# rickenator/steganosaurus

Hardware: AMD Instinct MI355X
Metric: MPixels/s embed+extract round-trip (RGB 2D-FFT fwd+inv) (higher is better)
Workload: dtype f32

## Files before the change

steganosaurus_amd/csrc/tfft_kernels.hip:

```cpp
#include <hip/hip_runtime.h>
#include <float.h>
#include <math.h>
#include <stdint.h>

#include <type_traits>

#include "tfft_fft.h"
#include "tfft_device.h"
#include "tfft_kernels.h"

#ifndef TFFT_WAVES_PER_EU
#define TFFT_WAVES_PER_EU(n) __attribute__((amdgpu_waves_per_eu(n)))
#endif
#ifndef TFFT_COLS_WAVES
#define TFFT_COLS_WAVES(logl) ((logl) >= 8 ? 4 : 1)
#endif
#ifndef TFFT_COLS_PF_MAXLOG
#define TFFT_COLS_PF_MAXLOG 7
#endif
#ifndef TFFT_COLS_PFEMIT
#define TFFT_COLS_PFEMIT 0
#endif
#ifndef TFFT_ROWS_LAZY_LOG
#define TFFT_ROWS_LAZY_LOG 11
// ... 636 lines not shown
            dstw[3 * g + 1] = G1 | (B1 << 8) | (R2 << 16) | (G2 << 24);
            dstw[3 * g + 2] = B2 | (R3 << 8) | (G3 << 16) | (B3 << 24);
        }
    } else {
        auto get = [&](int off) -> unsigned {
            const int n = off / 3, ch = off - 3 * n;
            float v = ldsf[2 * lay.idx(n >> 1, ch - plane0) + (n & 1)];
            if (P.center && ((n + y) & 1)) v = -v;
            return quantise_u8(v + (cov ? (float)cov[off] : P.bias));
        };
        if (PPB == 3) {
            const int head = (int)((4 - ((uintptr_t)dst & 3)) & 3);
            for (int o = tid; o < head && o < nbytes; o += nthr) dst[o] = (uint8_t)get(o);
            const int nwords = nbytes > head ? (nbytes - head) / 4 : 0;
            uint32_t* dstw = reinterpret_cast<uint32_t*>(dst + head);
            for (int w = tid; w < nwords; w += nthr) {
                const int o = head + 4 * w;
                dstw[w] = get(o) | (get(o + 1) << 8) | (get(o + 2) << 16) | (get(o + 3) << 24);
            }
            for (int o = head + 4 * nwords + tid; o < nbytes; o += nthr) dst[o] = (uint8_t)get(o);
        } else if ((P.W & 1) == 0) {
            const float s0 = (P.center && (y & 1)) ? -1.0f : 1.0f, s1 = P.center ? -s0 : s0;
            uint8_t* d1 = dst + plane0;
            constexpr int NP = imax(1, (M + T * PPB - 1) / (T * PPB));
            uint32_t cv[2 * NP];
            if (cov) {
#pragma unroll
                for (int i = 0; i < NP; i++) {
                    const uint8_t* a = cov + plane0 + 6 * imin(tid + i * nthr, (P.W >> 1) - 1);
                    cv[2 * i] = cover_word(a);
                    cv[2 * i + 1] = cover_word(a + 3);
                }
            }
#pragma unroll
            for (int i = 0; i < NP; i++) {
                const int m = tid + i * nthr;
                if (m >= (P.W >> 1)) break;
                const float2 v = lds[lay.idx(m, 0)];
                d1[6 * m] = (uint8_t)quantise_u8(s0 * v.x + (cov ? (float)cover_pick(cv[2 * i], cov + plane0 + 6 * m) : P.bias));
                d1[6 * m + 3] = (uint8_t)quantise_u8(s1 * v.y + (cov ? (float)cover_pick(cv[2 * i + 1], cov + plane0 + 6 * m + 3) : P.bias));
            }
        } else {
            for (int n = tid; n < P.W; n += nthr) dst[3 * n + plane0] = (uint8_t)get(3 * n + plane0);
        }
    }
}

__device__ __forceinline__ unsigned opaque_u32(unsigned v) {
#if defined(__HIPCC__)
    asm volatile("" : "+v"(v));
#endif
    return v;
}
constexpr int cols_threads(int logl) { return imax(256, 16 * ((1 << logl) / elems_for(1 << logl))); }
__device__ __forceinline__ int read_bit_value(float2 v, const EmbedParams& P, int p, const float* __restrict__ jitter, uint64_t j);

__device__ __forceinline__ unsigned frame_bit(const uint8_t* __restrict__ header, const uint8_t* __restrict__ payload, uint64_t i);
template <int LOGL, int SIGN, int MODE = COLS_PLAIN, bool DC = false, bool TW = false, bool FULL = false, bool PH = false, bool PI = false>
__global__ void __launch_bounds__(cols_threads(LOGL)) TFFT_WAVES_PER_EU((MODE == COLS_EMIT && TFFT_COLS_PFEMIT) ? 1 : (FULL ? TFFT_COLS_WAVES(LOGL) : imin(2, TFFT_COLS_WAVES(LOGL)))) k_fft_cols(const float2* in, float2* out, const float2* __restrict__ tw,
                           ColParams P) {
    constexpr int L = 1 << LOGL, E = elems_for(L), T = L / E, C = 16;
    constexpr bool STAT = stat_mode(MODE), FUSED = (MODE == COLS_STAT_EMBED);
    const int c = threadIdx.x, t = threadIdx.y, gl = (FUSED && T * C >= 256) ? 0 : (int)threadIdx.z;
    const int g = (MODE == COLS_PLAIN && SIGN > 0 && FULL && P.g_step > 1) ? (int)(blockIdx.y * blockDim.z + gl) * P.g_step + P.g_off
                                                                            : (int)(blockIdx.y * blockDim.z + gl);
    const int img = blockIdx.z / 3, plane = blockIdx.z - 3 * img;
    const size_t plane_off = (size_t)img * P.img_stride + (size_t)plane * P.plane_stride;
    float2* lds = reinterpret_cast<float2*>(tfft_smem) + (size_t)gl * L * C;
    LayColumns lay{C};

    if (MODE == COLS_PLAIN && SIGN > 0 && P.gate) {
        const SelectState* gs = P.gate + 3 * img;
        if (gs[0].fast && gs[1].fast && gs[2].fast && gs[0].n_amb <= TFFT_AMB_CAP && gs[1].n_amb <= TFFT_AMB_CAP && gs[2].n_amb <= TFFT_AMB_CAP) return;
    }
    const int ts = (MODE == COLS_PLAIN && SIGN > 0 && P.tile_step > 1) ? P.tile_step : 1;
    const int toff = ts > 1 ? P.tile_off : 0;
    const int tile0 = blockIdx.x * P.tiles_per_block;
    const int ntiles = ((P.M + C - 1) / C - toff + ts - 1) / ts;
    const int tile1 = (tile0 + P.tiles_per_block < ntiles) ? tile0 + P.tiles_per_block : ntiles;
    const int rows_in_max = P.in_a * (L - 1) + P.in_b * (P.G - 1);
    const bool in_full = (rows_in_max < P.in_rows) && (P.M % C == 0) && (P.G % (int)blockDim.z == 0);
    const unsigned voff_in = (unsigned)((P.in_a * t + P.in_b * g) * P.M + c) * 8u;
    const size_t stride_in = (size_t)P.in_a * T * P.M * sizeof(float2);
    const char* in_bytes = reinterpret_cast<const char*>(in + plane_off);
    const int oM = ts > 1 ? P.out_M : P.M;
    const unsigned voff_out = (unsigned)((P.out_a * t + P.out_b * g) * oM + c) * 8u;
    const size_t stride_out = (size_t)P.out_a * T * oM * sizeof(float2);
    char* out_bytes = reinterpret_cast<char*>(out + (ts > 1 ? (size_t)img * P.out_img_stride + (size_t)plane * P.out_plane_stride : plane_off));
    char* m2_bytes = reinterpret_cast<char*>(reinterpret_cast<float*>(out + (size_t)img * P.img_stride) + (size_t)plane * P.plane_stride);
    auto load_tile = [&](int tile, float2 (&v)[E]) {
        if (in_full) {
            const char* tb = in_bytes + (size_t)(imin(tile, ntiles - 1) * ts + toff) * (C * sizeof(float2));
            const unsigned vo = opaque_u32(voff_in);
#pragma unroll
            for (int m = 0; m < E; m++) v[m] = *reinterpret_cast<const float2*>(tb + m * stride_in + vo);
        } else {
            const int col = imin((tile * ts + toff) * C + c, P.M - 1);
            const float2* src = in + plane_off;
            const int gc = imin(g, P.G - 1), to = (int)opaque_u32((unsigned)t);
#pragma unroll
            for (int m = 0; m < E; m++) {
                const int row = imin(P.in_a * (to + m * T) + P.in_b * gc, P.in_rows - 1);
                v[m] = src[(unsigned)(row * P.M + col)];
            }
        }
    };
    auto tile_mask = [&](int tile, float2 (&v)[E]) {
        if (in_full) return;
        const bool active = ((tile * ts + toff) * C + c < P.M) && (g < P.G);
#pragma unroll
        for (int m = 0; m < E; m++) {
            const int row = P.in_a * (t + m * T) + P.in_b * g;
            if (!(active && row < P.in_rows)) v[m] = make_float2(0.f, 0.f);
        }
    };
    constexpr bool PF = (LOGL <= TFFT_COLS_PF_MAXLOG || (MODE == COLS_EMIT && TFFT_COLS_PFEMIT)) && !embed_mode(MODE);
    float2 u[E], un[E];
    float2 awc = make_float2(0.f, 0.f), awn = make_float2(0.f, 0.f);
    auto load_aw = [&](int tile) -> float2 { const int col = (tile * ts + toff) * C + c; return (DC && col < P.M) ? P.dc_aw[col] : make_float2(0.f, 0.f); };
    if (PF) { load_tile(tile0, u); awc = load_aw(tile0); }
    const int out_rows = (MODE == COLS_ROWLIMIT) ? imin(P.out_rows, *P.last_row_dev + 1) : P.out_rows;
    float2* lds_ah = reinterpret_cast<float2*>(tfft_smem) + (size_t)blockDim.z * L * C + (size_t)gl * L;
    float2* lds_wo = FUSED ? lds_ah : reinterpret_cast<float2*>(tfft_smem) + (size_t)blockDim.z * L * (C + (DC ? 1 : 0)) + (size_t)gl * L;
    auto fu_load_wo = [&]() -> float2 { return twload<-1>(tw, (int)((opaque_u32((unsigned)(t * C + c)) * (unsigned)g) & (unsigned)(P.PH - 1))); };
    auto fu_load_ah = [&]() -> float2 { return P.dc_ah[(unsigned)P.out_a * opaque_u32((unsigned)(t * C + c)) + (unsigned)(P.out_b * g)]; };
    if (FUSED && !DC) lds_wo[t * C + c] = fu_load_wo();
    if (DC) {
        for (int k = t * C + c; k < L; k += T * C) {
            const int row = (SIGN > 0) ? P.out_a * k + P.out_b * g : P.in_a * k + P.in_b * g;
            lds_ah[k] = (g < P.G && row < P.PH) ? P.dc_ah[row] : make_float2(0.f, 0.f);
        }
    }
    if (TW) {
        for (int k = t * C + c; k < L; k += T * C) lds_wo[k] = twload<SIGN>(tw, (k * g) & (P.PH - 1));
    }
    constexpr int NOFF = 16;
    constexpr bool TWL = (LOGL >= TFFT_COLS_LDS_TW_LOG) || FUSED;
    float2 W[TWL ? 1 : tw_regs<L, E>()];
    float2* lds_tw = reinterpret_cast<float2*>(tfft_smem) + (size_t)blockDim.z * L * (C + (DC || FUSED ? 1 : 0) + (TW ? 1 : 0));
    float2* lds_aw = lds_tw + (TWL ? L : 0) + gl * C;
    if (TWL) {
        const int tws = P.PH >> LOGL;
        for (int k = (gl * T + t) * C + c; k < L; k += blockDim.z * T * C) lds_tw[k] = tw[k * tws];
    } else {
        fft_prefetch_twiddles<L, E, SIGN>(W, t, tw, P.PH >> LOGL);
    }
#ifndef TFFT_EMBED_NE9
#ifndef TFFT_STAT_LDS_LOG
#define TFFT_STAT_LDS_LOG 9
#endif
#ifndef TFFT_STAT_SLOTS
#define TFFT_STAT_SLOTS 193
#endif
#define TFFT_EMBED_NE9 4
#endif
    constexpr int NE = (LOGL >= 9) ? (embed_mode(MODE) ? (LOGL == 9 ? TFFT_EMBED_NE9 : 2) : 4) : 2;
    struct EmEntry { TileBin tb; float2 f; unsigned bit, live; };
    EmEntry enC[NE], enN[NE];
    const int em_tid = t * C + c, em_nthr = T * C;
    unsigned* lds_eo = reinterpret_cast<unsigned*>(lds_tw + (TWL ? L : 0) + blockDim.z * C) + gl * (NOFF + 2);
    if (MODE == COLS_READ || embed_mode(MODE) || MODE == COLS_EMIT || STAT) {
        const unsigned b0 = (unsigned)(((PI ? (int)blockIdx.z : plane) * P.G + (g < P.G ? g : 0)) * ntiles);
        for (int i = em_tid; i <= NOFF; i += em_nthr) lds_eo[i] = P.rd_off[b0 + (unsigned)imin(tile0 + i, ntiles)];
    }
    unsigned* lds_hist = reinterpret_cast<unsigned*>(tfft_smem + P.hist_lds_off);
    const bool hist_on = (MODE == COLS_PLAIN && SIGN > 0 && FULL) && P.hist_sel != nullptr;
    if (hist_on)
        for (int i = (gl * T + t) * C + c; i < 4096; i += (int)(blockDim.x * blockDim.y * blockDim.z)) lds_hist[i] = 0;
    lds_barrier();
    auto em_range = [&](int tile, unsigned& e0, unsigned& e1) {
        const int i = imin(tile - tile0, NOFF - 1);
        e0 = lds_eo[i]; e1 = lds_eo[i + 1];
        if (!(tile < tile1 && g < P.G)) e1 = e0;
    };
    auto has_bins = [&](int tile) -> bool {
        if (MODE != COLS_READ || blockDim.z > 1) return true;
        unsigned e0, e1;
        em_range(tile, e0, e1);
        return e1 > e0;
    };
    const float2* em_fl = P.em_fl + (size_t)img * P.em_n;
    const uint8_t* em_pb = P.em_pb + (size_t)img * P.em_n;
    auto em_entries = [&](int tile, EmEntry (&en)[NE], bool with_value, bool with_bit) {
        unsigned e0, e1;
        em_range(tile, e0, e1);
#pragma unroll
        for (int i = 0; i < NE; i++) {
            const unsigned e = e0 + (unsigned)(em_tid + i * em_nthr);
            en[i].live = e < e1 ? 1u : 0u;
            const unsigned ec = en[i].live ? e : 0u;
            en[i].tb = P.rd_bins[ec];
            if (with_value) en[i].f = em_fl[ec];
            if (with_bit) en[i].bit = em_pb[ec];
        }
    };
    const float em_medp = (MODE == COLS_EMBED && PH && P.em_med) ? fmaxf(1e-12f, P.em_med[3 * img + plane]) : 1.f;
    auto em_delta = [&](float2 f, unsigned bit, unsigned conj, unsigned e) -> float2 {
        if (MODE == COLS_EMBED_D) return f;
        const float mag = fmaxf(1e-12f, mag_of(f));
        float ca = P.em_cos, sa = P.em_sin;
        if (MODE == COLS_EMBED && PH && P.em_med) sincosf(P.em_alpha * fminf(2.f, fmaxf(0.5f, mag / em_medp)), &sa, &ca);
        float2 nv = make_float2(mag * ca, bit ? mag * sa : -mag * sa);
        if (PH && P.em_jp) nv = cmul(nv, P.em_jp[e]);
        if (conj) nv = cconj(nv);
        return csub(nv, f);
    };
    const int st_lin = (gl * T + t) * C + c, st_wave = st_lin >> 6;
    unsigned* st_wbuf = lds_eo + (blockDim.z - gl) * (NOFF + 2) + st_wave * TFFT_STAT_SLOTS;
    SelectState* st_s = STAT ? P.st_sel + 3 * img + plane : nullptr;
    const unsigned st_lo = STAT ? st_s->lo : 0u, st_span = STAT ? st_s->hi - st_lo : 0u, st_base = st_lo << 19;
    const float st_t2lo = STAT ? fmaxf(st_s->t2_lo, 0.f) : 0.f, st_t2hi = STAT ? fmaxf(st_s->t2_hi, 0.f) : 0.f;
    unsigned* st_out = STAT ? P.st_cand + ((size_t)img * 3 + plane) * P.st_cand_stride : nullptr;
    float* st_ambo = STAT ? P.st_amb + ((size_t)img * 3 + plane) * TFFT_AMB_CAP : nullptr;
    unsigned st_below = 0, st_capcount = 0, st_nstaged = 0;
    const unsigned st_span_raw = st_span >= 8192u ? 0xFFFFFFFFu : ((st_span << 19) | 0x7FFFFu);
    const unsigned st_span_b = st_base > 0x7F800000u ? 0u : (st_span_raw < 0x7F800000u - st_base ? st_span_raw : 0x7F800000u - st_base);
    const unsigned st_aspan = (STAT && P.st_shi >= P.st_slo) ? P.st_shi - P.st_slo : 0u;
    const unsigned st_t2lo_b = __float_as_uint(st_t2lo), st_t2win = __float_as_uint(st_t2hi) - st_t2lo_b;
    unsigned* st_region = st_out + (size_t)(((blockIdx.y * gridDim.x + blockIdx.x) * ((blockDim.x * blockDim.y * blockDim.z + 63) >> 6)) + st_wave) * P.st_resv;
    if (STAT && blockIdx.x == 0 && blockIdx.y == 0 && st_lin == 0) st_s->cand_fixed = P.st_cand_fixed;
    unsigned st_used = 0;
    auto st_fill = [&]() {
        for (unsigned i = st_used + (st_lin & 63); i < P.st_resv; i += 64) st_region[i] = TFFT_CAND_HOLE;
    };
    auto st_flush = [&]() {
        const unsigned lane = st_lin & 63;
        WaveSync::sync();
        const unsigned room = P.st_resv - st_used, n1 = st_nstaged < room ? st_nstaged : room;
        for (unsigned i = lane; i < n1; i += 64) st_region[st_used + i] = st_wbuf[i];
        st_used += n1;
        if (st_nstaged > n1) {
            const unsigned rest = st_nstaged - n1;
            unsigned base = 0;
            if (lane == 0) base = atomicAdd(&st_s->n_cand, rest);
            base = __builtin_amdgcn_readfirstlane(base);
            if ((size_t)P.st_cand_fixed + base + rest <= P.st_cand_stride)
                for (unsigned i = lane; i < rest; i += 64) st_out[(size_t)P.st_cand_fixed + base + i] = st_wbuf[n1 + i];
        }
        WaveSync::sync();
        st_nstaged = 0;
    };
    if (embed_mode(MODE)) em_entries(tile0, enC, true, true);
    if (PF && (MODE == COLS_EMIT || STAT || MODE == COLS_READ)) em_entries(tile0, enC, false, FUSED);
    for (int tile = tile0; tile < tile1; tile++) {
        if (!PF && !embed_mode(MODE)) {
            if (!has_bins(tile)) continue;
            load_tile(tile, u); awc = load_aw(tile);
            if (MODE == COLS_EMIT || MODE == COLS_READ) em_entries(tile, enC, false, false);
        }
        if (PF) { const int nt = (tile + 1 < tile1 && has_bins(tile + 1)) ? tile + 1 : tile; load_tile(nt, un); awn = load_aw(nt); }
        if (PF && (MODE == COLS_EMIT || STAT || MODE == COLS_READ)) em_entries(tile + 1, enN, false, FUSED);
        if (embed_mode(MODE)) {
            bool hb = true;
            if (blockDim.z == 1) { unsigned e0, e1; em_range(tile, e0, e1); hb = e1 > e0; }
            em_entries(tile + 1, enN, true, true);
            if (hb) {
#pragma unroll
                for (int m = 0; m < E; m++) lds[lay.idx(t + m * T, c)] = make_float2(0.f, 0.f);
                lds_barrier();
                unsigned pe0 = 0;
                if (PH) { unsigned pe1; em_range(tile, pe0, pe1); }
#pragma unroll
                for (int i = 0; i < NE; i++)
                    if (enC[i].live && enC[i].bit < 2u)
                        lds[lay.idx(enC[i].tb.k, enC[i].tb.c)] = em_delta(enC[i].f, enC[i].bit, enC[i].tb.conj, pe0 + (unsigned)(em_tid + i * em_nthr));
                if (g < P.G) {
                    unsigned e0, e1;
                    em_range(tile, e0, e1);
                    for (unsigned e = e0 + (unsigned)(em_tid + NE * em_nthr); e < e1; e += em_nthr) {
                        const TileBin tb = P.rd_bins[e];
                        const unsigned bit = em_pb[e];
                        if (bit >= 2u) continue;
                        lds[lay.idx(tb.k, tb.c)] = em_delta(em_fl[e], bit, tb.conj, e);
                    }
                }
                lds_barrier();
#pragma unroll
                for (int m = 0; m < E; m++) u[m] = lds[lay.idx(t + m * T, c)];
                lds_barrier();
                if (TWL) fft_block_lazy<L, E, SIGN>(u, lds, lay, t, c, lds_tw, 1);
                else fft_block<L, E, SIGN>(u, lds, lay, t, c, W);
            }
                const int col = tile * C + c;
            if (FULL) {
                char* ob = out_bytes + (size_t)tile * (C * sizeof(float2));
                const unsigned vo = opaque_u32(voff_out);
#pragma unroll
                for (int m = 0; m < E; m++) {
                    float2 v = hb ? u[m] : make_float2(0.f, 0.f);
                    if (TW && hb) v = cmul(v, lds_wo[t + m * T]);
                    *reinterpret_cast<float2*>(ob + m * stride_out + vo) = v;
                }
            } else if ((col < P.M) && (g < P.G)) {
                float2* dst = out + plane_off;
                const int to = (int)opaque_u32((unsigned)t);
#pragma unroll
                for (int m = 0; m < E; m++) {
                    const int k = to + m * T;
                    const int row = P.out_a * k + P.out_b * g;
                    if (row < out_rows) {
                        float2 v = hb ? u[m] : make_float2(0.f, 0.f);
                        if (TW && hb) v = cmul(v, lds_wo[k]);
                        dst[(unsigned)(row * P.M + col)] = v;
                    }
                }
            }
#pragma unroll
            for (int i = 0; i < NE; i++) enC[i] = enN[i];
            continue;
        }
        if (PF && !has_bins(tile)) {
#pragma unroll
            for (int m = 0; m < E; m++) u[m] = un[m];
            awc = awn;
#pragma unroll
            for (int i = 0; i < NE; i++) enC[i] = enN[i];
            continue;
        }
        tile_mask(tile, u);
        if (DC && SIGN < 0) {
#pragma unroll
            for (int m = 0; m < E; m++) u[m] = csub(u[m], cmul(lds_ah[t + m * T], awc));
        }
        if (FUSED) fft_block_lazy<L, E, SIGN>(u, lds, lay, (int)opaque_u32((unsigned)t), c, lds_tw, 1);
        else if (TWL) fft_block_lazy<L, E, SIGN>(u, lds, lay, t, c, lds_tw, 1);
        else fft_block<L, E, SIGN>(u, lds, lay, t, c, W);
        if (MODE == COLS_READ) {
            lds_barrier();
#pragma unroll
            for (int m = 0; m < E; m++) lds[lay.idx(t + m * T, c)] = u[m];
            if (DC && t == 0) lds_aw[c] = awc;
            lds_barrier();
            if (FULL || g < P.G) {
                unsigned e0, e1;
                em_range(tile, e0, e1);
                uint8_t* bo = P.rd_bits + (size_t)img * P.rd_n;
                auto bit_of = [&](const TileBin tb, unsigned e) -> uint8_t {
                    float2 v = lds[lay.idx(tb.k, tb.c)];
                    if (DC) v = cadd(v, cmul(lds_ah[tb.k], lds_aw[tb.c]));
                    if (PH && P.em_jp) {
                        const float2 p = P.em_jp[e];
                        if (tb.conj) v = cconj(v);
                        return (uint8_t)(v.y * p.x - v.x * p.y >= 0.0f ? 1 : 0);
                    }
                    return (uint8_t)((tb.conj ? -v.y : v.y) >= 0.0f ? 1 : 0);
                };
#pragma unroll
                for (int i = 0; i < NE; i++) {
                    const TileBin tb = enC[i].tb;
                    uint8_t* dst = enC[i].live ? bo + tb.bit : P.trash + em_tid;
                    *dst = bit_of(tb, enC[i].live ? e0 + (unsigned)(em_tid + i * em_nthr) : 0u);
                }
                for (unsigned e = e0 + (unsigned)(em_tid + NE * em_nthr); e < e1; e += em_nthr) { const TileBin tb = P.rd_bins[e]; bo[tb.bit] = bit_of(tb, e); }
            }
            lds_barrier();
            if (PF) {
#pragma unroll
                for (int m = 0; m < E; m++) u[m] = un[m];
                awc = awn;
#pragma unroll
                for (int i = 0; i < NE; i++) enC[i] = enN[i];
            }
            continue;
        }
        const int col = tile * C + c;
        const bool st_valid = col != 0;
        const unsigned st_col2 = (unsigned)col * (unsigned)col, st_rstep = (unsigned)(P.out_a * T), st_row0 = opaque_u32((unsigned)(P.out_a * t + P.out_b * g));
        constexpr bool ST_LDS = (LOGL >= TFFT_STAT_LDS_LOG);
        unsigned st_ambflag = 0;
        auto st_value = [&](int m, float2 v) {
            const float m2 = st_valid ? fmaf(v.x, v.x, v.y * v.y) : -1.0f;
            const unsigned b = __float_as_uint(m2), rel = b - st_base, row = st_row0 + (unsigned)m * st_rstep;
            st_below += (b < st_base) ? 1u : 0u;
            const bool cnd = rel <= st_span_b;
            const unsigned long long mk = __ballot(cnd);
            {
                const unsigned slot = st_nstaged + wave_rank(mk), sel = (cnd && slot < (unsigned)(TFFT_STAT_SLOTS - 1)) ? 0xFFFFFFFFu : 0u;
                st_wbuf[(slot & sel) | ((unsigned)(TFFT_STAT_SLOTS - 1) & ~sel)] = rel | 0x80000000u;
                st_nstaged += (unsigned)__popcll(mk);
            }
            const unsigned d1 = __umul24(row, row) + st_col2;
            const float x = (d1 - P.st_slo <= st_aspan) ? m2 : -1.0f;
            st_capcount += !(x < st_t2hi) ? 1u : 0u;
            st_ambflag = st_ambflag + st_ambflag + ((__float_as_uint(x) - st_t2lo_b < st_t2win) ? 1u : 0u);
        };
        if (FULL && STAT && !ST_LDS) {
#ifndef TFFT_STAT_GROUP
#define TFFT_STAT_GROUP 8
#endif
#pragma unroll
            for (int m0 = 0; m0 < E; m0 += TFFT_STAT_GROUP) {
                float2 ahv[TFFT_STAT_GROUP];
#pragma unroll
                for (int j = 0; j < TFFT_STAT_GROUP; j++) ahv[j] = DC ? lds_ah[t + (m0 + j) * T] : make_float2(0.f, 0.f);
#pragma unroll
                for (int j = 0; j < TFFT_STAT_GROUP; j++) {
                    float2 v = u[m0 + j];
                    if (DC) v = cadd(v, cmul(ahv[j], awc));
                    st_value(m0 + j, v);
                }
            }
        } else if (FULL) {
            char* ob = out_bytes + (size_t)tile * (C * sizeof(float2));
            char* mb = m2_bytes + (size_t)tile * (C * sizeof(float));
            const unsigned vo = opaque_u32(voff_out);
#pragma unroll
            for (int m = 0; m < E; m++) {
                float2 v = u[m];
                if (TW) v = cmul(v, lds_wo[t + m * T]);
                if (DC && SIGN > 0) v = cadd(v, cmul(lds_ah[t + m * T], awc));
                if (STAT) {
                } else if (MODE == COLS_EMIT && P.em_m2) {
                    if (P.em_m2 == 1) *reinterpret_cast<float*>(mb + m * (stride_out >> 1) + (vo >> 1)) = fmaf(v.x, v.x, v.y * v.y);
                } else if (MODE == COLS_PLAIN && SIGN > 0 && hist_on) {
                    if ((tile * ts + toff) * C + c != 0) atomicAdd(&lds_hist[__float_as_uint(fmaf(v.x, v.x, v.y * v.y)) >> 19], 2u);
                } else *reinterpret_cast<float2*>(ob + m * stride_out + vo) = v;
            }
        } else if (((tile * ts + toff) * C + c < P.M) && (g < P.G)) {
            float2* dst = reinterpret_cast<float2*>(out_bytes);
            float* dst_m2 = reinterpret_cast<float*>(out + (size_t)img * P.img_stride) + (size_t)plane * P.plane_stride;
            const int to = (int)opaque_u32((unsigned)t);
#pragma unroll
            for (int m = 0; m < E; m++) {
                const int k = to + m * T;
                const int row = P.out_a * k + P.out_b * g;
                if (row < out_rows) {
                    float2 v = u[m];
                    if (TW) v = cmul(v, lds_wo[k]);
                    if (DC && SIGN > 0) v = cadd(v, cmul(lds_ah[k], awc));
                    if (MODE == COLS_EMIT && P.em_m2) {
                        if (P.em_m2 == 1) dst_m2[(unsigned)(row * P.M + col)] = fmaf(v.x, v.x, v.y * v.y);
                    } else dst[(unsigned)(row * oM + col)] = v;
                }
            }
        }
        if (((MODE == COLS_EMIT && P.em_m2 == 1) || STAT) && tile == 0 && c == 0 && g < P.G) {
            float2* col0 = P.st_col0 + ((size_t)img * 3 + plane) * P.PH;
            const int to = (int)opaque_u32((unsigned)t);
#pragma unroll
            for (int m = 0; m < E; m++) {
                const int row = P.out_a * (to + m * T) + P.out_b * g;
                if (row < out_rows) col0[(unsigned)row] = (DC && SIGN > 0) ? cadd(u[m], cmul(lds_ah[to + m * T], awc)) : u[m];
            }
        }
        if (MODE == COLS_EMIT || STAT) {
            lds_barrier();
#pragma unroll
            for (int m = 0; m < E; m++) lds[lay.idx(t + m * T, c)] = u[m];
            if (DC && t == 0) lds_aw[c] = awc;
            lds_barrier();
            float2 fu_wo = make_float2(0.f, 0.f);
            if (FUSED && DC) fu_wo = fu_load_wo();
            if (STAT) {
                if (ST_LDS) {
#pragma unroll 4
                    for (int m = 0; m < E; m++) {
                        const int k = t + m * T;
                        float2 v = lds[lay.idx(k, c)];
                        if (DC) v = cadd(v, cmul(lds_ah[k], awc));
                        st_value(m, v);
                    }
                }
                {
                    auto st_again = [&](int m, float& m2, unsigned& row) -> bool {
                        const int k = t + m * T;
                        float2 v = lds[lay.idx(k, c)];
                        if (DC) v = cadd(v, cmul(lds_ah[k], awc));
                        m2 = fmaf(v.x, v.x, v.y * v.y);
                        row = st_row0 + (unsigned)m * st_rstep;
                        return row * row + st_col2 - P.st_slo <= st_aspan;
                    };
                    auto st_uncount = [&](int m) {
                        float m2; unsigned row;
                        if (st_again(m, m2, row) && !(m2 < st_t2hi)) st_capcount -= 1u;
                    };
                    const unsigned half = (unsigned)P.PH >> 1, dh = half - st_row0;
                    if (st_valid && st_row0 == 0) st_uncount(0);
                    if (st_valid && half != 0 && half >= st_row0 && dh % st_rstep == 0 && dh / st_rstep < (unsigned)E) st_uncount((int)(dh / st_rstep));
                    if (st_nstaged > (unsigned)(TFFT_STAT_SLOTS - 1)) {
                        st_nstaged = 0;
                        for (int m = 0; m < E; m++) {
                            float m2; unsigned row;
                            (void)st_again(m, m2, row);
                            const unsigned rel = __float_as_uint(st_valid ? m2 : -1.0f) - st_base;
                            const bool cnd = rel <= st_span_b;
                            const unsigned long long mk = __ballot(cnd);
                            if (cnd) st_wbuf[st_nstaged + wave_rank(mk)] = rel | 0x80000000u;
                            st_nstaged += (unsigned)__popcll(mk);
                            if (st_nstaged > 64) st_flush();
                        }
                    }
                    if (st_nstaged) st_flush();
                    if (__ballot(st_ambflag != 0)) {
                        for (int m = 0; m < E; m++) {
                            if (!((st_ambflag >> (E - 1 - m)) & 1u)) continue;
                            float m2; unsigned row;
                            if (st_again(m, m2, row) && !(m2 < st_t2lo) && m2 < st_t2hi && row != 0 && 2u * row != (unsigned)P.PH) {
                                const unsigned slot = atomicAdd(&st_s->n_amb, 1u);
                                if (slot < TFFT_AMB_CAP) st_ambo[slot] = m2;
                            }
                        }
                    }
                }
            }
            if (!PF && STAT) em_entries(tile, enC, false, FUSED);
            auto read_listed = [&](const TileBin tb) -> float2 {
                float2 v = lds[lay.idx(tb.k, tb.c)];
                if (DC) v = cadd(v, cmul(lds_ah[tb.k], lds_aw[tb.c]));
                return v;
            };
            if constexpr (FUSED) {
                unsigned e0, e1;
                em_range(tile, e0, e1);
                bool hb = true;
                if (blockDim.z == 1) hb = e1 > e0;
                if (hb) {
                    float2* fl = P.em_fl + (size_t)img * P.em_n;
#pragma unroll
                    for (int i = 0; i < NE; i++) {
                        const TileBin tb = enC[i].tb;
                        enC[i].f = read_listed(tb);
                    }
                    for (unsigned e = e0 + (unsigned)(em_tid + NE * em_nthr); e < e1; e += em_nthr) {
                        const TileBin tb = P.rd_bins[e];
                        fl[e] = read_listed(tb);
                    }
                    lds_barrier();
#pragma unroll
                    for (int m = 0; m < E; m++) lds[lay.idx(t + m * T, c)] = make_float2(0.f, 0.f);
                    if (DC) lds_wo[t * C + c] = fu_wo;
                    lds_barrier();
#pragma unroll
                    for (int i = 0; i < NE; i++)
                        if (enC[i].live && enC[i].bit < 2u)
                            lds[lay.idx(enC[i].tb.k, enC[i].tb.c)] = em_delta(enC[i].f, enC[i].bit, enC[i].tb.conj, e0 + (unsigned)(em_tid + i * em_nthr));
                    for (unsigned e = e0 + (unsigned)(em_tid + NE * em_nthr); e < e1; e += em_nthr) {
                        const TileBin tb = P.rd_bins[e];
                        const unsigned bit = em_pb[e];
                        if (bit >= 2u) continue;
                        lds[lay.idx(tb.k, tb.c)] = em_delta(em_fl[e], bit, tb.conj, e);
                    }
                    lds_barrier();
#pragma unroll
                    for (int m = 0; m < E; m++) u[m] = lds[lay.idx(t + m * T, c)];
                    lds_barrier();
                    fft_block_lazy<L, E, -1>(u, lds, lay, (int)opaque_u32((unsigned)t), c, lds_tw, 1);
                }
                char* ob = out_bytes + (size_t)tile * (C * sizeof(float2));
                const unsigned vo = opaque_u32(voff_in);
                float2 fu_ah = make_float2(0.f, 0.f);
                if (DC) fu_ah = fu_load_ah();
#pragma unroll
                for (int m = 0; m < E; m++) {
                    float2 v = make_float2(0.f, 0.f);
                    if (hb) v = cmul(u[m], lds_wo[t + m * T]);
                    *reinterpret_cast<float2*>(ob + m * stride_in + vo) = v;
                }
                static_assert(!FUSED || LOGL >= TFFT_TILE_FUSE_MIN_LOG, "COLS_STAT_EMBED: from L = 32 on");
                if (DC && hb) {
                    lds_barrier();
                    lds_ah[t * C + c] = fu_ah;
                } else if (!hb) lds_barrier();
            } else {
                unsigned e0, e1;
                em_range(tile, e0, e1);
                float2* fl = P.em_fl + (size_t)img * P.em_n;
#pragma unroll
                for (int i = 0; i < NE; i++) {
                    const TileBin tb = enC[i].tb;
                    float2* dst = enC[i].live ? fl + (e0 + (unsigned)(em_tid + i * em_nthr)) : reinterpret_cast<float2*>(P.trash) + em_tid;
                    *dst = read_listed(tb);
                }
                for (unsigned e = e0 + (unsigned)(em_tid + NE * em_nthr); e < e1; e += em_nthr) {
                    const TileBin tb = P.rd_bins[e];
                    fl[e] = read_listed(tb);
                }
                lds_barrier();
            }
            if (PF) {
#pragma unroll
                for (int i = 0; i < NE; i++) enC[i] = enN[i];
            }
        }
        if (PF) {
#pragma unroll
            for (int m = 0; m < E; m++) u[m] = un[m];
            awc = awn;
        }
    }
    if (MODE == COLS_PLAIN && SIGN > 0 && FULL) {
        if (hist_on) {
            lds_barrier();
            unsigned* gh = P.hist_sel[3 * img + plane].hist;
            for (int i = (gl * T + t) * C + c; i < 4096; i += (int)(blockDim.x * blockDim.y * blockDim.z))
                if (lds_hist[i]) atomicAdd(&gh[i], lds_hist[i]);
        }
    }
    if (STAT) {
        unsigned* st_wcnt = lds_eo + (blockDim.z - opaque_u32(threadIdx.z)) * (NOFF + 2) + ((blockDim.x * blockDim.y * blockDim.z + 63) >> 6) * TFFT_STAT_SLOTS;
        st_fill();
        lds_barrier();
        if (threadIdx.x == 0 && threadIdx.y == 0 && threadIdx.z == 0) { st_wcnt[0] = 0; st_wcnt[1] = 0; }
        lds_barrier();
        if (st_below) atomicAdd(&st_wcnt[0], 2u * st_below);
        if (st_capcount) atomicAdd(&st_wcnt[1], st_capcount);
        lds_barrier();
        if (threadIdx.x == 0 && threadIdx.y == 0 && threadIdx.z == 0) {
            if (st_wcnt[0]) atomicAdd(&st_s->below, (unsigned long long)st_wcnt[0]);
            if (P.st_cap && st_wcnt[1])
                atomicAdd(&P.st_partial[((size_t)img * 3 + plane) * TFFT_STAT_MAX_BLOCKS + ((blockIdx.y * gridDim.x + blockIdx.x) % TFFT_STAT_MAX_BLOCKS)], st_wcnt[1]);
        }
    }
}

struct BinRef { size_t idx; bool conj; };
__device__ __forceinline__ BinRef locate(int plane, int y, int x, int PH, int PW) {
    const int M = PW >> 1;
    if (x < M) return BinRef{((size_t)plane * PH + y) * M + x, false};
    const int yy = (PH - y) & (PH - 1);
    return BinRef{((size_t)plane * PH + yy) * M + (PW - x), true};
}
__device__ __forceinline__ float2 full_bin(const float2* __restrict__ plane, int y, int x, int PH, int PW) {
    const int M = PW >> 1;
    if (x == 0 || x == M) {
        float2 f0, fm; unpack_col0(plane, y, PH, M, f0, fm);
        return x == 0 ? f0 : fm;
    }
    if (x < M) return plane[(size_t)y * M + x];
    return cconj(plane[(size_t)((PH - y) & (PH - 1)) * M + (PW - x)]);
}

__global__ void k_bins_last_row(const tfft_bin* __restrict__ bins, uint64_t n, int PH, int PW, int* __restrict__ last_row) {
    int* blk = reinterpret_cast<int*>(tfft_smem);
    if (threadIdx.x == 0) blk[0] = 0;
    __syncthreads();
    int mine = 0;
    for (uint64_t i = (uint64_t)blockIdx.x * blockDim.x + threadIdx.x; i < n; i += (uint64_t)gridDim.x * blockDim.x) {
        const tfft_bin bn = bins[i];
        const int x = bn.x, y = bn.y;
        if (x >= PW || y >= PH) continue;
        const int row = (x <= (PW >> 1)) ? y : ((PH - y) & (PH - 1));
        mine = row > mine ? row : mine;
    }
    if (mine) atomicMax(&blk[0], mine);
    __syncthreads();
    if (threadIdx.x == 0 && blk[0]) atomicMax(last_row, blk[0]);
}

__device__ __forceinline__ unsigned frame_bit(const uint8_t* __restrict__ header, const uint8_t* __restrict__ payload, uint64_t i) {
    uint64_t b; const uint8_t* src;
    if (i < 912) { b = i / 3; src = header; }
    else { b = (i - 912) / 7; src = payload; }
    return (unsigned)((src[b >> 3] >> (7 - (b & 7))) & 1);
}

__global__ void k_embed(float2* __restrict__ spec, const tfft_bin* __restrict__ bins, const uint8_t* __restrict__ bits,
                        const float* __restrict__ jitter, EmbedParams P, int* __restrict__ err) {
    const uint64_t i = (uint64_t)blockIdx.x * blockDim.x + threadIdx.x;
    if (i >= P.n) return;
    const int img = blockIdx.y;
    spec += (size_t)img * P.img_stride;
    if (bits) bits += (size_t)img * P.n;
    bins += (size_t)img * P.bins_stride;
// ... 670 lines not shown
        Q.tiles_per_block = tpb;
    }
    const size_t nwaves = ((size_t)C * T * gpb + 63) / 64;
    const size_t lds = lds0 + (BUCKETS ? (size_t)gpb * (C * sizeof(float2) + 18 * sizeof(unsigned)) : 0) +
                       (stat_mode(MODE) ? (nwaves * (TFFT_STAT_SLOTS + 1) + 2) * sizeof(unsigned) : 0);
    size_t lds_total = lds;
    if (MODE == COLS_PLAIN && SIGN > 0 && P.hist_sel) {
        if (!FULL) return hipErrorInvalidValue;
        Q.hist_lds_off = (unsigned)((lds + 15) & ~(size_t)15);
        lds_total = Q.hist_lds_off + 4096 * sizeof(unsigned);
    }
    if (gsample && (!FULL || P.g_off + (Geff - 1) * P.g_step >= P.G)) return hipErrorInvalidValue;
    dim3 grid((ntiles + tpb - 1) / tpb, (Geff + gpb - 1) / gpb, n_planes), block(C, T, gpb);
    if (stat_mode(MODE)) {
        Q.st_resv = 64u * (unsigned)tpb;
        const size_t fixed = (size_t)grid.x * grid.y * nwaves * Q.st_resv;
        if (fixed + (size_t)P.PH * (P.M + 1) > P.st_cand_stride) return hipErrorInvalidValue;
        Q.st_cand_fixed = (unsigned)fixed;
    }
    if constexpr (MODE == COLS_STAT_EMBED && !FULL) return hipErrorInvalidValue;
    else {
        auto k = k_fft_cols<LOGL, SIGN, MODE, DC, TW, FULL, PH, PI>;
        if (lds_total > 48 * 1024) {
            hipError_t e = hipFuncSetAttribute((const void*)k, hipFuncAttributeMaxDynamicSharedMemorySize, (int)lds_total);
            if (e != hipSuccess) return e;
        }
        hipLaunchKernelGGL(k, grid, block, lds_total, s, in, out, tw, Q);
        return hipGetLastError();
    }
}
constexpr bool cols_variant_exists(int mode, int sign, bool dc, bool tw, bool ph, bool pi) {
    if (sign < 0) return mode == COLS_PLAIN ? !ph && !pi : mode == COLS_EMBED ? !dc : mode == COLS_EMBED_D ? !dc && !ph && pi : false;
    switch (mode) {
        case COLS_PLAIN: return !(dc && tw) && !ph && !pi;
        case COLS_ROWLIMIT: return !tw && !ph && !pi;
        case COLS_READ: return !tw;
        case COLS_EMIT: case COLS_STAT: return !tw && !ph;
        case COLS_STAT_EMBED: return !tw;
        default: return false;
    }
}
template <int LO, int HI, class F>
static hipError_t with_constant(int v, const F& f) {
    if constexpr (LO > HI) return hipErrorInvalidValue;
    else return v == LO ? f(std::integral_constant<int, LO>{}) : with_constant<LO + 1, HI>(v, f);
}
hipError_t launch_cols(const float2* in, float2* out, const float2* tw_ph, const ColParams& P, const ColStep& step, int n_planes, hipStream_t s) {
    const int mode = step.mode;
    const bool fwd = step.sign > 0, emit = mode == COLS_EMIT || stat_mode(mode), buckets = emit || embed_mode(mode) || mode == COLS_READ;
    if (step.logl > 9) return hipErrorInvalidValue;
    if (buckets && (!P.rd_bins || !P.trash)) return hipErrorInvalidValue;
    if ((emit || embed_mode(mode)) && !P.em_fl) return hipErrorInvalidValue;
    if (mode == COLS_ROWLIMIT && !P.last_row_dev) return hipErrorInvalidValue;
    if (mode == COLS_STAT_EMBED && (!fwd || !P.em_pb || P.em_m2 || in == out || P.in_a != 1 || P.in_b != (1 << step.logl) || P.out_b != 1)) return hipErrorInvalidValue;
    if (stat_mode(mode) && (step.logl < 4 || !P.st_sel || !P.st_cand || !P.st_col0 || (P.st_cap && (!P.st_partial || !P.st_amb)))) return hipErrorInvalidValue;
    if (P.em_m2 && fwd && !(emit && P.st_col0)) return hipErrorInvalidValue;
    if ((P.tile_step > 1 || P.gate) && !(mode == COLS_PLAIN && fwd && !P.tw_out)) return hipErrorInvalidValue;
    if (P.em_med && mode != COLS_EMBED) return hipErrorInvalidValue;
    const int sw = (P.dc_ah ? 1 : 0) | (P.tw_out ? 2 : 0) | (P.em_jp || P.em_med ? 4 : 0) | (step.walks ? 8 : 0);
    return with_constant<0, 9>(step.logl, [&](auto logl) {
        return with_constant<0, 1>(fwd ? 1 : 0, [&](auto f) {
            return with_constant<COLS_PLAIN, COLS_STAT_EMBED>(mode, [&](auto m) {
                return with_constant<0, 15>(sw, [&](auto w) {
                    constexpr int LOGL = decltype(logl)::value, SIGN = decltype(f)::value ? +1 : -1, MODE = decltype(m)::value, SW = decltype(w)::value;
                    constexpr bool DC = SW & 1, TW = SW & 2, PH = SW & 4, PI = SW & 8;
                    if constexpr (cols_variant_exists(MODE, SIGN, DC, TW, PH, PI) && !(MODE == COLS_STAT_EMBED && LOGL < TFFT_TILE_FUSE_MIN_LOG)) return launch_cols_t<LOGL, SIGN, MODE, DC, TW, false, PH, PI>(in, out, tw_ph, P, n_planes, s);
                    else return hipErrorInvalidValue;
                });
            });
        });
    });
}

hipError_t launch_bucket_bins(const tfft_bin* bins, const uint32_t* bit_index, uint64_t n, int PH, int PW, int G,
                              unsigned* cnt, unsigned* off, TileBin* out, int* err, int force_global, hipStream_t s) {
    const int M = PW >> 1, ntiles = (M + 15) >> 4, nb = 3 * ntiles * G;
    hipError_t e = hipMemsetAsync(cnt, 0, (size_t)nb * sizeof(unsigned), s);
    if (e != hipSuccess) return e;
    unsigned blocks = (unsigned)((n + 2047) / 2048);
    if (blocks < 1) blocks = 1;
    if (blocks > 4096) blocks = 4096;
    const size_t lds = (BUCKET_LCAP + 2) * sizeof(unsigned);
    hipLaunchKernelGGL(k_bucket_count, dim3(blocks), dim3(256), lds, s, bins, n, PH, PW, G, cnt, err, force_global);
    const int nblk = (nb + 1023) / 1024;
    if (nblk > 1024) return hipErrorInvalidValue;
    unsigned* totals = off + nb + 1;
    hipLaunchKernelGGL(k_bucket_scan_a, dim3(nblk), dim3(1024), 1024 * sizeof(unsigned), s, cnt, off, totals, nb);
    hipLaunchKernelGGL(k_bucket_scan_b, dim3(1), dim3(1024), 1024 * sizeof(unsigned), s, totals, nblk, off, nb);
    hipLaunchKernelGGL(k_bucket_scan_c, dim3(nblk), dim3(1024), 0, s, off, totals, nb);
    hipLaunchKernelGGL(k_bucket_fill, dim3(blocks), dim3(256), lds, s, bins, bit_index, n, PH, PW, G, cnt, off, out, force_global);
    return hipGetLastError();
}
hipError_t launch_bucket_walks(const tfft_bin* bins, uint64_t n, int n_images, int PH, int PW, int G, unsigned* cnt, unsigned* off, TileBin* out,
                               int* err, hipStream_t s) {
    if (n == 0 || n_images <= 0) return hipErrorInvalidValue;
    const int M = PW >> 1, ntiles = (M + 15) >> 4;
    const unsigned nb = 3u * (unsigned)ntiles * (unsigned)G, nbi = nb + 1;
    const uint64_t nbt = (uint64_t)nb * (uint64_t)n_images + 1;
    if (nbt > 1024ull * 1024ull || (uint64_t)n * (uint64_t)n_images > 0xFFFFFFFFull) return hipErrorInvalidValue;
    hipError_t e = hipMemsetAsync(cnt, 0, (size_t)nbt * sizeof(unsigned), s);
    if (e != hipSuccess) return e;
    int chunks = (int)((n + 8191) / 8192);
    if (chunks < 1) chunks = 1;
    if ((uint64_t)chunks * (uint64_t)n_images > 65535ull) chunks = 65535 / n_images > 0 ? 65535 / n_images : 1;
    const size_t lds = nbi <= BUCKET_LCAP ? (size_t)nbi * sizeof(unsigned) : 16;
    hipLaunchKernelGGL(k_bucket_count_walks, dim3((unsigned)(chunks * n_images)), dim3(256), lds, s, bins, n, chunks, PH, PW, G, nb, cnt, err);
    const int nblk = (int)((nbt + 1023) / 1024);
// ... 730 lines not shown
```

Baseline: 25530.

## Use buffer resource loads/stores and kernarg-reloaded cold params in column FFT kernel

Replaces 64-bit pointer arithmetic for column tile loads and stores with AMDGPU raw buffer loads and stores that take a scalar resource descriptor plus 32-bit offsets, so per-element address math needs fewer vector registers. Rarely used stat pointers are re-read from the kernarg segment through the constant address space and kept in scalar registers, instead of being held live for the whole kernel. The fused stat-embed path is assumed to be in-bounds, which drops its masking, and a matching launch check is added. The risks are possible 32-bit offset overflow on large planes and a different register and scheduling profile.

Result: faster. 25790, median of 6 (+1.0%).

```diff
diff --git a/steganosaurus_amd/csrc/tfft_kernels.hip b/steganosaurus_amd/csrc/tfft_kernels.hip
--- a/steganosaurus_amd/csrc/tfft_kernels.hip
+++ b/steganosaurus_amd/csrc/tfft_kernels.hip
@@ -712,6 +712,68 @@
 #endif
     return v;
 }
+struct PlaneBuf {
+#if defined(__HIPCC__)
+    __amdgpu_buffer_rsrc_t rs;
+#else
+    char* base;
+#endif
+};
+__device__ __forceinline__ PlaneBuf plane_buf(const void* base, size_t bytes) {
+    PlaneBuf b;
+#if defined(__HIPCC__)
+    b.rs = __builtin_amdgcn_make_buffer_rsrc(const_cast<void*>(base), 0, (int)bytes, 0x00020000);
+#else
+    (void)bytes;
+    b.base = reinterpret_cast<char*>(const_cast<void*>(base));
+#endif
+    return b;
+}
+__device__ __forceinline__ float2 plane_load(const PlaneBuf& b, unsigned voff, unsigned soff) {
+#if defined(__HIPCC__)
+    const auto r = __builtin_amdgcn_raw_buffer_load_b64(b.rs, (int)voff, (int)soff, 0);
+    return make_float2(__uint_as_float(r[0]), __uint_as_float(r[1]));
+#else
+    return *reinterpret_cast<const float2*>(b.base + (size_t)soff + voff);
+#endif
+}
+__device__ __forceinline__ void plane_store(const PlaneBuf& b, unsigned voff, unsigned soff, float2 v) {
+#if defined(__HIPCC__)
+    typedef unsigned v2u __attribute__((ext_vector_type(2)));
+    v2u r;
+    r[0] = __float_as_uint(v.x); r[1] = __float_as_uint(v.y);
+    __builtin_amdgcn_raw_buffer_store_b64(r, b.rs, (int)voff, (int)soff, 0);
+#else
+    *reinterpret_cast<float2*>(b.base + (size_t)soff + voff) = v;
+#endif
+}
+__device__ __forceinline__ void plane_store(const PlaneBuf& b, unsigned voff, unsigned soff, float v) {
+#if defined(__HIPCC__)
+    __builtin_amdgcn_raw_buffer_store_b32(__float_as_uint(v), b.rs, (int)voff, (int)soff, 0);
+#else
+    *reinterpret_cast<float*>(b.base + (size_t)soff + voff) = v;
+#endif
+}
+#if defined(__HIPCC__)
+typedef const __attribute__((address_space(4))) ColParams* ColdParams;
+#else
+typedef const ColParams* ColdParams;
+#endif
+__device__ __forceinline__ unsigned cold_u32(unsigned v) {
+#if defined(__HIPCC__)
+    asm volatile("" : "+s"(v));
+#endif
+    return v;
+}
+__device__ __forceinline__ ColdParams cold_params(const ColParams& P) {
+#if defined(__HIPCC__)
+    uint64_t k = (uint64_t)__builtin_amdgcn_kernarg_segment_ptr();
+    asm volatile("" : "+s"(k));
+    return (ColdParams)(k + 3 * sizeof(void*));
+#else
+    return &P;
+#endif
+}
 constexpr int cols_threads(int logl) { return imax(256, 16 * ((1 << logl) / elems_for(1 << logl))); }
 __device__ __forceinline__ int read_bit_value(float2 v, const EmbedParams& P, int p, const float* __restrict__ jitter, uint64_t j);
 
@@ -739,21 +801,24 @@
     const int ntiles = ((P.M + C - 1) / C - toff + ts - 1) / ts;
     const int tile1 = (tile0 + P.tiles_per_block < ntiles) ? tile0 + P.tiles_per_block : ntiles;
     const int rows_in_max = P.in_a * (L - 1) + P.in_b * (P.G - 1);
-    const bool in_full = (rows_in_max < P.in_rows) && (P.M % C == 0) && (P.G % (int)blockDim.z == 0);
+    const bool in_full = (FUSED && T * C >= 256) || ((rows_in_max < P.in_rows) && (P.M % C == 0) && (P.G % (int)blockDim.z == 0));
+    const bool g_in = FULL || g < P.G;
     const unsigned voff_in = (unsigned)((P.in_a * t + P.in_b * g) * P.M + c) * 8u;
-    const size_t stride_in = (size_t)P.in_a * T * P.M * sizeof(float2);
-    const char* in_bytes = reinterpret_cast<const char*>(in + plane_off);
+    const unsigned stride_in = (unsigned)(P.in_a * T * P.M) * (unsigned)sizeof(float2);
     const int oM = ts > 1 ? P.out_M : P.M;
     const unsigned voff_out = (unsigned)((P.out_a * t + P.out_b * g) * oM + c) * 8u;
-    const size_t stride_out = (size_t)P.out_a * T * oM * sizeof(float2);
+    const unsigned stride_out = (unsigned)(P.out_a * T * oM) * (unsigned)sizeof(float2);
     char* out_bytes = reinterpret_cast<char*>(out + (ts > 1 ? (size_t)img * P.out_img_stride + (size_t)plane * P.out_plane_stride : plane_off));
-    char* m2_bytes = reinterpret_cast<char*>(reinterpret_cast<float*>(out + (size_t)img * P.img_stride) + (size_t)plane * P.plane_stride);
+    const PlaneBuf in_buf = plane_buf(in + plane_off, (size_t)P.PH * P.M * sizeof(float2));
+    const PlaneBuf out_buf = plane_buf(out_bytes, (size_t)P.PH * oM * sizeof(float2));
+    const PlaneBuf m2_buf = plane_buf(reinterpret_cast<float*>(out + (size_t)img * P.img_stride) + (size_t)plane * P.plane_stride,
+                                      (size_t)P.PH * P.M * sizeof(float));
     auto load_tile = [&](int tile, float2 (&v)[E]) {
         if (in_full) {
-            const char* tb = in_bytes + (size_t)(imin(tile, ntiles - 1) * ts + toff) * (C * sizeof(float2));
+            const unsigned so = (unsigned)(imin(tile, ntiles - 1) * ts + toff) * (unsigned)(C * sizeof(float2));
             const unsigned vo = opaque_u32(voff_in);
 #pragma unroll
-            for (int m = 0; m < E; m++) v[m] = *reinterpret_cast<const float2*>(tb + m * stride_in + vo);
+            for (int m = 0; m < E; m++) v[m] = plane_load(in_buf, vo, so + (unsigned)m * stride_in);
         } else {
             const int col = imin((tile * ts + toff) * C + c, P.M - 1);
             const float2* src = in + plane_off;
@@ -767,10 +832,11 @@
     };
     auto tile_mask = [&](int tile, float2 (&v)[E]) {
         if (in_full) return;
-        const bool active = ((tile * ts + toff) * C + c < P.M) && (g < P.G);
+        const bool active = ((tile * ts + toff) * C + c < P.M) && g_in;
+        const int to = FULL ? (int)opaque_u32((unsigned)t) : t;
 #pragma unroll
         for (int m = 0; m < E; m++) {
-            const int row = P.in_a * (t + m * T) + P.in_b * g;
+            const int row = P.in_a * (to + m * T) + P.in_b * g;
             if (!(active && row < P.in_rows)) v[m] = make_float2(0.f, 0.f);
         }
     };
@@ -788,7 +854,7 @@
     if (DC) {
         for (int k = t * C + c; k < L; k += T * C) {
             const int row = (SIGN > 0) ? P.out_a * k + P.out_b * g : P.in_a * k + P.in_b * g;
-            lds_ah[k] = (g < P.G && row < P.PH) ? P.dc_ah[row] : make_float2(0.f, 0.f);
+            lds_ah[k] = (g_in && row < P.PH) ? P.dc_ah[row] : make_float2(0.f, 0.f);
         }
     }
     if (TW) {
@@ -820,7 +886,7 @@
     const int em_tid = t * C + c, em_nthr = T * C;
     unsigned* lds_eo = reinterpret_cast<unsigned*>(lds_tw + (TWL ? L : 0) + blockDim.z * C) + gl * (NOFF + 2);
     if (MODE == COLS_READ || embed_mode(MODE) || MODE == COLS_EMIT || STAT) {
-        const unsigned b0 = (unsigned)(((PI ? (int)blockIdx.z : plane) * P.G + (g < P.G ? g : 0)) * ntiles);
+        const unsigned b0 = (unsigned)(((PI ? (int)blockIdx.z : plane) * P.G + (g_in ? g : 0)) * ntiles);
         for (int i = em_tid; i <= NOFF; i += em_nthr) lds_eo[i] = P.rd_off[b0 + (unsigned)imin(tile0 + i, ntiles)];
     }
     unsigned* lds_hist = reinterpret_cast<unsigned*>(tfft_smem + P.hist_lds_off);
@@ -831,7 +897,7 @@
     auto em_range = [&](int tile, unsigned& e0, unsigned& e1) {
         const int i = imin(tile - tile0, NOFF - 1);
         e0 = lds_eo[i]; e1 = lds_eo[i + 1];
-        if (!(tile < tile1 && g < P.G)) e1 = e0;
+        if (!(tile < tile1 && g_in)) e1 = e0;
     };
     auto has_bins = [&](int tile) -> bool {
         if (MODE != COLS_READ || blockDim.z > 1) return true;
@@ -868,16 +934,16 @@
     const int st_lin = (gl * T + t) * C + c, st_wave = st_lin >> 6;
     unsigned* st_wbuf = lds_eo + (blockDim.z - gl) * (NOFF + 2) + st_wave * TFFT_STAT_SLOTS;
     SelectState* st_s = STAT ? P.st_sel + 3 * img + plane : nullptr;
+    auto st_state = [&]() -> SelectState* { return cold_params(P)->st_sel + cold_u32(blockIdx.z); };
+    auto st_list = [&]() -> unsigned* { ColdParams Q = cold_params(P); return Q->st_cand + (size_t)cold_u32(blockIdx.z) * Q->st_cand_stride; };
     const unsigned st_lo = STAT ? st_s->lo : 0u, st_span = STAT ? st_s->hi - st_lo : 0u, st_base = st_lo << 19;
     const float st_t2lo = STAT ? fmaxf(st_s->t2_lo, 0.f) : 0.f, st_t2hi = STAT ? fmaxf(st_s->t2_hi, 0.f) : 0.f;
-    unsigned* st_out = STAT ? P.st_cand + ((size_t)img * 3 + plane) * P.st_cand_stride : nullptr;
-    float* st_ambo = STAT ? P.st_amb + ((size_t)img * 3 + plane) * TFFT_AMB_CAP : nullptr;
     unsigned st_below = 0, st_capcount = 0, st_nstaged = 0;
     const unsigned st_span_raw = st_span >= 8192u ? 0xFFFFFFFFu : ((st_span << 19) | 0x7FFFFu);
     const unsigned st_span_b = st_base > 0x7F800000u ? 0u : (st_span_raw < 0x7F800000u - st_base ? st_span_raw : 0x7F800000u - st_base);
     const unsigned st_aspan = (STAT && P.st_shi >= P.st_slo) ? P.st_shi - P.st_slo : 0u;
     const unsigned st_t2lo_b = __float_as_uint(st_t2lo), st_t2win = __float_as_uint(st_t2hi) - st_t2lo_b;
-    unsigned* st_region = st_out + (size_t)(((blockIdx.y * gridDim.x + blockIdx.x) * ((blockDim.x * blockDim.y * blockDim.z + 63) >> 6)) + st_wave) * P.st_resv;
+    unsigned* st_region = (STAT ? P.st_cand + ((size_t)img * 3 + plane) * P.st_cand_stride : nullptr) + (size_t)(((blockIdx.y * gridDim.x + blockIdx.x) * ((blockDim.x * blockDim.y * blockDim.z + 63) >> 6)) + st_wave) * P.st_resv;
     if (STAT && blockIdx.x == 0 && blockIdx.y == 0 && st_lin == 0) st_s->cand_fixed = P.st_cand_fixed;
     unsigned st_used = 0;
     auto st_fill = [&]() {
@@ -892,10 +958,14 @@
         if (st_nstaged > n1) {
             const unsigned rest = st_nstaged - n1;
             unsigned base = 0;
-            if (lane == 0) base = atomicAdd(&st_s->n_cand, rest);
+            if (lane == 0) base = atomicAdd(&st_state()->n_cand, rest);
             base = __builtin_amdgcn_readfirstlane(base);
-            if ((size_t)P.st_cand_fixed + base + rest <= P.st_cand_stride)
-                for (unsigned i = lane; i < rest; i += 64) st_out[(size_t)P.st_cand_fixed + base + i] = st_wbuf[n1 + i];
+            ColdParams Q = cold_params(P);
+            const size_t fixed = Q->st_cand_fixed;
+            if (fixed + base + rest <= Q->st_cand_stride) {
+                unsigned* st_out = st_list();
+                for (unsigned i = lane; i < rest; i += 64) st_out[fixed + base + i] = st_wbuf[n1 + i];
+            }
         }
         WaveSync::sync();
         st_nstaged = 0;
@@ -924,7 +994,7 @@
                 for (int i = 0; i < NE; i++)
                     if (enC[i].live && enC[i].bit < 2u)
                         lds[lay.idx(enC[i].tb.k, enC[i].tb.c)] = em_delta(enC[i].f, enC[i].bit, enC[i].tb.conj, pe0 + (unsigned)(em_tid + i * em_nthr));
-                if (g < P.G) {
+                if (g_in) {
                     unsigned e0, e1;
                     em_range(tile, e0, e1);
                     for (unsigned e = e0 + (unsigned)(em_tid + NE * em_nthr); e < e1; e += em_nthr) {
@@ -943,13 +1013,13 @@
             }
                 const int col = tile * C + c;
             if (FULL) {
-                char* ob = out_bytes + (size_t)tile * (C * sizeof(float2));
+                const unsigned so = (unsigned)tile * (unsigned)(C * sizeof(float2));
                 const unsigned vo = opaque_u32(voff_out);
 #pragma unroll
                 for (int m = 0; m < E; m++) {
                     float2 v = hb ? u[m] : make_float2(0.f, 0.f);
                     if (TW && hb) v = cmul(v, lds_wo[t + m * T]);
-                    *reinterpret_cast<float2*>(ob + m * stride_out + vo) = v;
+                    plane_store(out_buf, vo, so + (unsigned)m * stride_out, v);
                 }
             } else if ((col < P.M) && (g < P.G)) {
                 float2* dst = out + plane_off;
@@ -991,7 +1061,7 @@
             for (int m = 0; m < E; m++) lds[lay.idx(t + m * T, c)] = u[m];
             if (DC && t == 0) lds_aw[c] = awc;
             lds_barrier();
-            if (FULL || g < P.G) {
+            if (g_in) {
                 unsigned e0, e1;
                 em_range(tile, e0, e1);
                 uint8_t* bo = P.rd_bits + (size_t)img * P.rd_n;
@@ -1061,8 +1131,7 @@
                 }
             }
         } else if (FULL) {
-            char* ob = out_bytes + (size_t)tile * (C * sizeof(float2));
-            char* mb = m2_bytes + (size_t)tile * (C * sizeof(float));
+            const unsigned so = (unsigned)tile * (unsigned)(C * sizeof(float2));
             const unsigned vo = opaque_u32(voff_out);
 #pragma unroll
             for (int m = 0; m < E; m++) {
@@ -1071,10 +1140,10 @@
                 if (DC && SIGN > 0) v = cadd(v, cmul(lds_ah[t + m * T], awc));
                 if (STAT) {
                 } else if (MODE == COLS_EMIT && P.em_m2) {
-                    if (P.em_m2 == 1) *reinterpret_cast<float*>(mb + m * (stride_out >> 1) + (vo >> 1)) = fmaf(v.x, v.x, v.y * v.y);
+                    if (P.em_m2 == 1) plane_store(m2_buf, vo >> 1, (so >> 1) + (unsigned)m * (stride_out >> 1), fmaf(v.x, v.x, v.y * v.y));
                 } else if (MODE == COLS_PLAIN && SIGN > 0 && hist_on) {
                     if ((tile * ts + toff) * C + c != 0) atomicAdd(&lds_hist[__float_as_uint(fmaf(v.x, v.x, v.y * v.y)) >> 19], 2u);
-                } else *reinterpret_cast<float2*>(ob + m * stride_out + vo) = v;
+                } else plane_store(out_buf, vo, so + (unsigned)m * stride_out, v);
             }
         } else if (((tile * ts + toff) * C + c < P.M) && (g < P.G)) {
             float2* dst = reinterpret_cast<float2*>(out_bytes);
@@ -1094,8 +1163,8 @@
                 }
             }
         }
-        if (((MODE == COLS_EMIT && P.em_m2 == 1) || STAT) && tile == 0 && c == 0 && g < P.G) {
-            float2* col0 = P.st_col0 + ((size_t)img * 3 + plane) * P.PH;
+        if (((MODE == COLS_EMIT && P.em_m2 == 1) || STAT) && tile == 0 && c == 0 && g_in) {
+            float2* col0 = cold_params(P)->st_col0 + (size_t)cold_u32(blockIdx.z) * P.PH;
             const int to = (int)opaque_u32((unsigned)t);
 #pragma unroll
             for (int m = 0; m < E; m++) {
@@ -1156,8 +1225,8 @@
                             if (!((st_ambflag >> (E - 1 - m)) & 1u)) continue;
                             float m2; unsigned row;
                             if (st_again(m, m2, row) && !(m2 < st_t2lo) && m2 < st_t2hi && row != 0 && 2u * row != (unsigned)P.PH) {
-                                const unsigned slot = atomicAdd(&st_s->n_amb, 1u);
-                                if (slot < TFFT_AMB_CAP) st_ambo[slot] = m2;
+                                const unsigned slot = atomicAdd(&st_state()->n_amb, 1u);
+                                if (slot < TFFT_AMB_CAP) (cold_params(P)->st_amb + (size_t)cold_u32(blockIdx.z) * TFFT_AMB_CAP)[slot] = m2;
                             }
                         }
                     }
@@ -1206,7 +1275,7 @@
                     lds_barrier();
                     fft_block_lazy<L, E, -1>(u, lds, lay, (int)opaque_u32((unsigned)t), c, lds_tw, 1);
                 }
-                char* ob = out_bytes + (size_t)tile * (C * sizeof(float2));
+                const unsigned so = (unsigned)tile * (unsigned)(C * sizeof(float2));
                 const unsigned vo = opaque_u32(voff_in);
                 float2 fu_ah = make_float2(0.f, 0.f);
                 if (DC) fu_ah = fu_load_ah();
@@ -1214,7 +1283,7 @@
                 for (int m = 0; m < E; m++) {
                     float2 v = make_float2(0.f, 0.f);
                     if (hb) v = cmul(u[m], lds_wo[t + m * T]);
-                    *reinterpret_cast<float2*>(ob + m * stride_in + vo) = v;
+                    plane_store(out_buf, vo, so + (unsigned)m * stride_in, v);
                 }
                 static_assert(!FUSED || LOGL >= TFFT_TILE_FUSE_MIN_LOG, "COLS_STAT_EMBED: from L = 32 on");
                 if (DC && hb) {
@@ -1251,7 +1320,7 @@
     if (MODE == COLS_PLAIN && SIGN > 0 && FULL) {
         if (hist_on) {
             lds_barrier();
-            unsigned* gh = P.hist_sel[3 * img + plane].hist;
+            unsigned* gh = cold_params(P)->hist_sel[cold_u32(blockIdx.z)].hist;
             for (int i = (gl * T + t) * C + c; i < 4096; i += (int)(blockDim.x * blockDim.y * blockDim.z))
                 if (lds_hist[i]) atomicAdd(&gh[i], lds_hist[i]);
         }
@@ -1266,9 +1335,10 @@
         if (st_capcount) atomicAdd(&st_wcnt[1], st_capcount);
         lds_barrier();
         if (threadIdx.x == 0 && threadIdx.y == 0 && threadIdx.z == 0) {
-            if (st_wcnt[0]) atomicAdd(&st_s->below, (unsigned long long)st_wcnt[0]);
-            if (P.st_cap && st_wcnt[1])
-                atomicAdd(&P.st_partial[((size_t)img * 3 + plane) * TFFT_STAT_MAX_BLOCKS + ((blockIdx.y * gridDim.x + blockIdx.x) % TFFT_STAT_MAX_BLOCKS)], st_wcnt[1]);
+            ColdParams Q = cold_params(P);
+            if (st_wcnt[0]) atomicAdd(&st_state()->below, (unsigned long long)st_wcnt[0]);
+            if (Q->st_cap && st_wcnt[1])
+                atomicAdd(&Q->st_partial[(size_t)cold_u32(blockIdx.z) * TFFT_STAT_MAX_BLOCKS + ((blockIdx.y * gridDim.x + blockIdx.x) % TFFT_STAT_MAX_BLOCKS)], st_wcnt[1]);
         }
     }
 }
@@ -2045,7 +2115,7 @@
     if (buckets && (!P.rd_bins || !P.trash)) return hipErrorInvalidValue;
     if ((emit || embed_mode(mode)) && !P.em_fl) return hipErrorInvalidValue;
     if (mode == COLS_ROWLIMIT && !P.last_row_dev) return hipErrorInvalidValue;
-    if (mode == COLS_STAT_EMBED && (!fwd || !P.em_pb || P.em_m2 || in == out || P.in_a != 1 || P.in_b != (1 << step.logl) || P.out_b != 1)) return hipErrorInvalidValue;
+    if (mode == COLS_STAT_EMBED && (!fwd || !P.em_pb || P.em_m2 || in == out || P.in_a != 1 || P.in_b != (1 << step.logl) || P.out_b != 1 || (P.G << step.logl) > P.in_rows)) return hipErrorInvalidValue;
     if (stat_mode(mode) && (step.logl < 4 || !P.st_sel || !P.st_cand || !P.st_col0 || (P.st_cap && (!P.st_partial || !P.st_amb)))) return hipErrorInvalidValue;
     if (P.em_m2 && fwd && !(emit && P.st_col0)) return hipErrorInvalidValue;
     if ((P.tile_step > 1 || P.gate) && !(mode == COLS_PLAIN && fwd && !P.tw_out)) return hipErrorInvalidValue;
```
